# lincbrain/Fibers.jl

Hardware: AMD Instinct MI355X
Metric: Mvoxels/s fit (GQI ODF + peaks, 140^3 x 270-dir); Mpoints/s streamline in extra (higher is better)
Workload: dtype f32 (operands as 2 fp16 pieces = 23 bits on MFMA, 3 piece products, f32 accumulate); 1 GPU; gqi_rec + find_peaks + qa normalisation (gqi.jl:109-201), ONE 140x140x140 x 270-frame volume (18 x b=5 + 84 dirs x {1000,2000,3000}), sphere_642, all-ones mask; voxels=2744000, voxels_per_gpu=2744000, frames=270, odf_vertices=321, parallelism=single GPU

## Files before the change

fibers.jl_amd/csrc/odf.hip:

```cpp
#include <algorithm>
#include <cmath>
#include <type_traits>
#include <utility>

#include "common.h"

namespace {

typedef float f32x16 __attribute__((ext_vector_type(16)));

constexpr int KT = 16;
constexpr int WG_VOX = 128;

#include "odf_gemm_f32.inc"
#include "odf_fused_epilogue.inc"
#include "odf_gemm3.inc"
#include "odf_mask.inc"
#include "odf_peaks.inc"
#include "odf_post.inc"

}

struct fib_odf_plan {
    int device = 0, ncu = 256;
    int nvol = 0, nvert = 0, nrows = 0, nrow0 = 0;
    int MB = 11, NX = 0, ntile_m = 1, Kpad = 0, maxdeg = 0;
    int scale_frame = -1;
    float scale_coef = 0.0f;
    bool has_ineff = false;
    int gM = 0, gK = 0, gRow0 = 0;
    std::vector<float> G;
    bool folded = false;
    int fold_span_max = 0, scale_frame_raw = -1;
    fib::DevBuf<int32_t> foldA, foldB;
    mutable fib::DevBuf<float> folded_dwi;
    std::vector<float> A;
    fib::DevBuf<float> At, verts;
    fib::DevBuf<uint16_t> At3;
    fib::DevBuf<float> Aextra;
    fib::DevBuf<float> Gdev;
    mutable fib::DevBuf<int32_t> inf_list;
    bool split_bf16 = false;
    bool h2 = false;
    float h2_sa = 1.0f;
    bool fused_shape = false;
    bool fused = false;
    bool dsi2_shape = false, dsi2 = false;
    int MBB = 0;
    fib::DevBuf<uint16_t> At3b;
    mutable fib::DevBuf<unsigned> pair_flags;
    fib::DevBuf<uint16_t> At3f;
    fib::DevBuf<float> Aextraf;
    mutable fib::DevBuf<float> mean_hi;
    mutable fib::DevBuf<int32_t> redo_list;
    fib::DevBuf<uint32_t> effbits;
    fib::DevBuf<int32_t> nbr, nbr64;
    int deg_pad = 6, rows_pad = 0;
// ... 3 lines not shown
    mutable fib::DevBuf<unsigned long long> compact_state;
    mutable fib::DevBuf<unsigned long long> compact_sub;
    mutable fib::DevBuf<unsigned long long> compact_state2;
    mutable fib::DevBuf<unsigned> compact_mode;
    mutable fib::DevBuf<unsigned long long> compact_oct;
    mutable unsigned compact_epoch = 0;
    fib::DevBuf<unsigned> tickets;
    fib::DevBuf<unsigned> selctr;
    fib::DevBuf<unsigned long long> sellist;
    mutable fib::DevBuf<float> odfmax;
};

namespace {


int resolve_format(int format) {
    if (format != FIB_ODF_FORMAT_DEFAULT) return format;
    const char *e = fib::env("FIBERS_ODF_FORMAT");
    if (!e) {
        const char *g = fib::env("FIBERS_ODF_GEMM"), *x = fib::env("FIBERS_ODF_EXACT");
        if (g && (!strcmp(g, "f32") || !strcmp(g, "F32"))) return FIB_ODF_FORMAT_F32;
        if (x && x[0] != '\0' && x[0] != '0') return FIB_ODF_FORMAT_BF16X3;
    }
    if (e && (!strcmp(e, "f32") || !strcmp(e, "F32"))) return FIB_ODF_FORMAT_F32;
    if (e && (!strcmp(e, "bf16x3") || !strcmp(e, "BF16X3"))) return FIB_ODF_FORMAT_BF16X3;
    return FIB_ODF_FORMAT_FP16X2;
}

int finish_plan(fib_odf_plan *p, const float *verts, int nverts, const int32_t *faces, int nfaces,
                const std::vector<float> &frame_eff, int format = FIB_ODF_FORMAT_DEFAULT) {
    if (p->G.empty()) { p->G = p->A; p->gM = p->nrows; p->gK = p->nvol; p->gRow0 = p->nrow0; }
    const int M = p->gM, K = p->gK;
    if (hipDeviceGetAttribute(&p->ncu, hipDeviceAttributeMultiprocessorCount, p->device) != hipSuccess) p->ncu = 256;
    format = resolve_format(format);
    p->split_bf16 = format != FIB_ODF_FORMAT_F32;
    int best_cost = INT32_MAX;
    const int nxs[] = {0, 1};
    for (int mb = p->split_bf16 ? 10 : 11; mb >= 5; mb--)
        for (int nx : nxs) {
            if (nx > 0 && mb > 10) continue;
            const int rows = mb * 32 + nx;
            const int nt = (M + rows - 1) / rows;
            const int cost = nt * (64 * mb + 4 * nx);
            if (cost < best_cost) { best_cost = cost; p->MB = mb; p->NX = nx; p->ntile_m = nt; }
        }
    p->Kpad = (K + KT - 1) / KT * KT;
    const int MW = gemm_row_stride(p->MB, p->NX), ROWS = p->MB * 32 + p->NX;
    std::vector<float> At((size_t)p->ntile_m * p->Kpad * MW, 0.0f);
    for (int k = 0; k < K; k++)
        for (int r = 0; r < M; r++) {
            const int tm = r / ROWS, rr = r % ROWS;
            At[((size_t)tm * p->Kpad + k) * MW + rr] = p->G[r + (size_t)M * k];
        }
    bool any_ineff = false;
    for (int k = 0; k < K; k++) if (frame_eff[k] == 0.0f) any_ineff = true;
    if (p->split_bf16 && (any_ineff || p->Kpad / KT < 2 || p->MB > 10 || (size_t)p->ntile_m * p->NX * p->Kpad > 2048)) p->split_bf16 = false;
    if (p->split_bf16) {
        p->h2 = format == FIB_ODF_FORMAT_FP16X2;
        float gmax = 0.0f;
        for (float v : p->G) if (std::isfinite(v)) gmax = std::max(gmax, std::fabs(v));
        if (p->h2 && !(gmax > 0.0f)) p->h2 = false;
        for (float v : p->G) if (!std::isfinite(v)) p->h2 = false;
        if (p->h2) { int eg; std::frexp(gmax, &eg); p->h2_sa = std::ldexp(1.0f, 9 - eg); }
        const int NP = p->h2 ? 2 : 3;
        const int npiece = NP * p->MB, nst = p->Kpad / KT;
        auto f16_rn = [](float f) -> uint16_t { const _Float16 h = (_Float16)f; uint16_t u; memcpy(&u, &h, 2); return u; };
// ... 232 lines not shown
                if (fa[c] == p->scale_frame) p->scale_frame = -1000 - c;
            }
            if (p->scale_frame <= -1000) { p->scale_frame = -(p->scale_frame + 1000); p->scale_frame_raw = fa[p->scale_frame]; }
            for (int t0 = 0; t0 < nrep; t0 += KT)
                for (const std::vector<int32_t> *side : {&fa, &fb}) {
                    int lo = 1 << 30, hi = -1;
                    for (int j = t0; j < std::min(nrep, t0 + KT); j++) if ((*side)[j] >= 0) { lo = std::min(lo, (*side)[j]); hi = std::max(hi, (*side)[j]); }
                    if (hi >= 0) p->fold_span_max = std::max(p->fold_span_max, hi - lo + 1);
                }
            FIB_RC(fib::upload(p->foldA, fa));
            FIB_RC(fib::upload(p->foldB, fb));
            eff.assign((size_t)nrep, 1.0f);
        }
    }
    FIB_RC(finish_plan(p.get(), verts, nverts, faces, nfaces, eff, format));
    *plan = p.release();
    return FIB_OK;
} FIB_API_CATCH

extern "C" void fib_odf_plan_destroy(fib_odf_plan *plan) try { fib::plan_destroy(plan); } FIB_API_CATCH_VOID

extern "C" int fib_odf_plan_matrix(const fib_odf_plan *plan, float *A, int *nrows, int *nvol, int *nvert) try {
    FIB_CHECK(plan != nullptr, FIB_ERR_INVALID, "plan is NULL");
    if (nrows) *nrows = plan->nrows;
    if (nvol) *nvol = plan->nvol;
    if (nvert) *nvert = plan->nvert;
    if (A) memcpy(A, plan->A.data(), plan->A.size() * sizeof(float));
    return FIB_OK;
} FIB_API_CATCH

namespace {

constexpr int FOLD_MB_MAX = 10;
constexpr int POST_GRID = 384;

struct OdfRoute {
    bool compact = false;
    bool split = false;
    bool fused = false;
    bool dsi2 = false;
    bool fold_fused = false;
    bool fold_pre = false;
    bool fold4 = false;
    bool inf_fix = false;
    bool peaks = false;
    bool vec_ok = false;
    bool scan() const { return fused || dsi2; }
};

OdfRoute odf_route(const fib_odf_plan *plan, int64_t nvox, bool out16, bool in16, int flags) {
    OdfRoute r;
    const bool sep = (flags & FIB_ODF_SEPARATE_PEAKS) != 0;
    r.compact = true;
    r.vec_ok = out16;
    r.split = plan->split_bf16 && nvox <= ((int64_t)1 << 26);
    r.inf_fix = r.split && plan->Gdev.p != nullptr;
    r.fused = plan->fused && r.split && out16 && !sep;
    const bool fold_ok = plan->folded && r.split && plan->Kpad <= FKMAX && plan->scale_frame_raw >= 0 &&
                         (int64_t)plan->fold_span_max * nvox * 4 < (int64_t)0xE0000000ll;
    r.dsi2 = plan->dsi2 && fold_ok && out16 && !sep;
    r.fold_fused = (fold_ok && plan->MB <= FOLD_MB_MAX) || r.dsi2;
    r.fold_pre = plan->folded && !r.fold_fused;
    r.fold4 = r.fold_pre && in16;
    r.peaks = !r.scan();
    return r;
}

// ... 170 lines not shown
    return FIB_OK;
}

int launch_mask_compact(const fib_odf_plan *plan, const uint8_t *mask, int64_t nvox, unsigned *maxenc, const ZeroArgs *z, hipStream_t st) {
    int iters = (int)std::max<int64_t>(1, fib::cdiv(fib::cdiv(nvox, CB), 256));
    if (iters > CB_ITERS_MAX) iters = CB_ITERS_MAX;
    const int nchunks = (int)fib::cdiv(nvox, (int64_t)CB * iters);
    FIB_CHECK(nchunks <= 1024, FIB_ERR_UNSUPPORTED, "volume too large for the mask compaction");
    FIB_RC(fresh_zeroed(plan->compact_state, 1024, st));
    FIB_RC(fresh_zeroed(plan->compact_state2, 1024, st));
    if (!plan->compact_mode.p) {
        FIB_RC(plan->compact_mode.alloc(2));
        FIB_HIP(hipMemsetD32Async(reinterpret_cast<hipDeviceptr_t>(plan->compact_mode.p), 1, 2, st));
    }
    if (z) FIB_RC(fresh_zeroed(plan->compact_sub, (size_t)fib::cdiv(nvox, CB), st));
    if (++plan->compact_epoch == 0u) plan->compact_epoch = 1u;
    CompactArgs c{};
    c.mask = mask; c.nvox = nvox; c.vidx = plan->live_vox.p; c.tiles = plan->live_tiles.p; c.state = plan->compact_state.p;
    c.ticket = plan->tickets.p; c.totals = plan->live_counts.p; c.maxenc = maxenc; c.epoch = plan->compact_epoch; c.nchunks = nchunks; c.iters = iters;
    c.zero = z != nullptr;
    if (z) c.z = *z;
    c.clear = plan->pair_flags.p; c.nclear = plan->pair_flags.p ? 8 * 32 : 0;
    c.sub_state = plan->compact_sub.p;
    c.state2 = plan->compact_state2.p; c.mode = plan->compact_mode.p;
    const size_t noct = (size_t)fib::cdiv(nvox, 1024);
    if (z && noct * sizeof(unsigned) <= 48 * 1024) {
        FIB_RC(fresh_zeroed(plan->compact_oct, noct, st));
        c.oct_bits = plan->compact_oct.p; c.oct_words = (int)noct;
    }
    { const char *e = fib::ab_env("FIBERS_COMPACT_UNKNOWN"); c.dbg_unknown = e ? atoi(e) : 0; }
    { const char *e = fib::ab_env("FIBERS_ODF_LIST"); c.force = !e ? -1 : (e[0] == 'q' ? 0 : (e[0] == 'o' ? 1 : -1)); }
    fib::ProfScope prof("mask_compact", st);
    const int grid = nchunks + (z ? 256 : 0);
    hipLaunchKernelGGL(mask_compact_kernel, dim3(grid), dim3(1024), c.oct_words * sizeof(unsigned), st, c);
    FIB_HIP(hipGetLastError());
    return FIB_OK;
}

void launch_fold(const fib_odf_plan *plan, const OdfRoute &r, const float *dwi, const uint8_t *mask, int64_t nvox, hipStream_t st) {
    fib::ProfScope prof("dsi_fold", st);
    const unsigned grid = (unsigned)fib::cdiv(r.fold4 ? nvox / 4 : nvox, 256);
    hipLaunchKernelGGL(r.fold4 ? dsi_fold4_kernel : dsi_fold_kernel, dim3(grid), dim3(256), 0, st, dwi, mask, plan->foldA.p, plan->foldB.p,
                       plan->gK, nvox, plan->folded_dwi.p);
}

GemmArgs odf_gemm_args(const fib_odf_plan *plan, const OdfRoute &r, const float *dwi, const uint8_t *mask, float *pdf, float *odf,
                       float *const peak[3], float *const qa[3], int64_t nvox) {
    GemmArgs ga = gemm_args(plan, r, r.fold_pre ? plan->folded_dwi.p : dwi, mask, pdf, odf, nvox);
#ifdef FIB_CLOCK_STAMP
    { const char *pi = fib::ab_env("FIBERS_PHASE_ITEM"); ga.phase_item = pi ? atoi(pi) : 2; }
    { const char *pw = fib::ab_env("FIBERS_PHASE_WG"); ga.phase_wg = pw ? atoi(pw) : 8; }
#endif
    if (r.inf_fix) { ga.fix_count = plan->live_counts.p + 2; ga.fix_list = plan->inf_list.p; ga.fix_cap = (int)std::min<int64_t>(nvox, INT32_MAX); }
    if (r.scan()) add_scan_args(ga, plan, peak, qa);
    if (r.dsi2) add_dsi2_args(ga, plan);
    return ga;
}

int launch_post(const fib_odf_plan *plan, const OdfRoute &r, const GemmArgs &ga, const float *dwi, float *odf, float *const peak[3],
                float *const qa[3], int64_t nvox, float *odfmax, int flags, hipStream_t st) {
    fib::ProfScope prof("odf_post", st);
    PostArgs pa{};
    pa.redo = RedoArgs{odf, nvox, ga.redo_count, ga.redo_list, ga.redo_cap, plan->verts.p, {peak[0], peak[1], peak[2]}, {qa[0], qa[1], qa[2]}, plan->maxenc.p};
    pa.G = (r.scan() && r.inf_fix) ? plan->Gdev.p : nullptr; pa.S = dwi; pa.out = odf; pa.M = plan->gM; pa.K = plan->gK;
    pa.refine = RefineArgs{odf, nvox, nvox, plan->nvert, plan->live_vox.p, plan->live_counts.p, plan->mean_hi.p, plan->maxenc.p};
    pa.arrive = plan->tickets.p + 1; pa.odfmax = odfmax; pa.raw = (flags & FIB_ODF_RAW_ODFMAX) ? 1 : 0;
    pa.selctr = plan->selctr.p; pa.sellist = plan->sellist.p; pa.selcap = POST_SELCAP; pa.epoch = plan->compact_epoch;
    if (flags & FIB_ODF_NORMALIZE) {
        for (int k = 0; k < 3; k++) pa.nq[k] = qa[k];
        pa.nq_n = nvox; pa.done = reinterpret_cast<unsigned long long *>(plan->tickets.p + 2);
    }
    { const char *e = fib::ab_env("FIBERS_POST_SKIP"); pa.dbg = e ? atoi(e) : 0; }
    hipLaunchKernelGGL(odf_post_kernel, dim3(POST_GRID), dim3(256), 0, st, pa);
    FIB_HIP(hipGetLastError());
    return FIB_OK;
}
}

extern "C" int fibd_odf_rec(const fib_odf_plan *plan, const float *dwi, const uint8_t *mask, int64_t nvox,
                            float *pdf, float *odf, float *const peak[3], float *const qa[3],
                            float *odfmax_dev, int flags, void *stream) try {
    FIB_CHECK(plan && dwi && mask && odf && peak && qa, FIB_ERR_INVALID, "NULL argument");
    FIB_CHECK(nvox > 0, FIB_ERR_INVALID, "nvox must be positive");
    FIB_CHECK(nvox <= ((int64_t)1 << 27), FIB_ERR_UNSUPPORTED, "volumes of more than 2^27 voxels are not supported (32-bit lane offsets)");
    FIB_CHECK(plan->nrow0 == 0 || pdf != nullptr, FIB_ERR_INVALID, "DSI plans need a pdf output volume");
    for (int k = 0; k < 3; k++) FIB_CHECK(peak[k] && qa[k], FIB_ERR_INVALID, "NULL peak/qa output volume");
    FIB_CHECK(fib::cdiv(nvox, WG_VOX) * plan->ntile_m < ((int64_t)1 << 31), FIB_ERR_UNSUPPORTED, "volume too large for one launch");
    fib::DeviceGuard guard;
    FIB_HIP(hipSetDevice(plan->device));
    hipStream_t st = (hipStream_t)stream;
    const bool out16 = nvox % 4 == 0 && ((uintptr_t)odf & 15) == 0 && (pdf == nullptr || ((uintptr_t)pdf & 15) == 0);
    const bool in16 = nvox % 4 == 0 && ((uintptr_t)dwi & 15) == 0 && ((uintptr_t)mask & 3) == 0;
    const OdfRoute route = odf_route(plan, nvox, out16, in16, flags);
    FIB_RC(odf_scratch(plan, route, nvox));
    ZeroArgs z{};
    z.out0 = pdf; z.out1 = odf; z.n0 = plan->nrow0; z.n1 = plan->nrows - plan->nrow0; z.nvox = nvox; z.stride = nvox;
    for (int k = 0; k < 3; k++) { z.peak[k] = peak[k]; z.qa[k] = qa[k]; }
    FIB_RC(launch_mask_compact(plan, mask, nvox, plan->maxenc.p, !(flags & FIB_ODF_PREZEROED) ? &z : nullptr, st));
    if (route.fold_pre) launch_fold(plan, route, dwi, mask, nvox, st);
    const GemmArgs ga = odf_gemm_args(plan, route, dwi, mask, pdf, odf, peak, qa, nvox);
    FIB_RC(launch_contraction(plan, route, ga, "odf_gemm", st));
    if (route.peaks) {
        if (route.inf_fix) {
            InfFixArgs fx{plan->Gdev.p, dwi, odf, ga.fix_count, ga.fix_list, ga.fix_cap, plan->gM, plan->gK, nvox};
            hipLaunchKernelGGL(odf_inf_fix_kernel, dim3(64), dim3(256), 0, st, fx);
        }
        FIB_RC(launch_peaks(plan, odf, nvox, nvox, peak, qa, nullptr, nullptr, true, st, false, plan->live_tiles.p, plan->live_counts.p + 1));
// ... 48 lines not shown

extern "C" int fibd_qa_normalize_dev(float *const qa[3], int64_t nvox, const float *odfmax_dev, void *stream) try {
    FIB_CHECK(qa && qa[0] && qa[1] && qa[2] && odfmax_dev && nvox > 0, FIB_ERR_INVALID, "NULL argument");
    return qa_normalize(qa, nvox, const_cast<float *>(odfmax_dev), 0.0f, 0, stream);
} FIB_API_CATCH

extern "C" int fibd_qa_normalize_pair(float *const qa[3], int64_t nvox, float *odfmax_pair_dev, void *stream) try {
    FIB_CHECK(qa && qa[0] && qa[1] && qa[2] && odfmax_pair_dev && nvox > 0, FIB_ERR_INVALID, "NULL argument");
    return qa_normalize(qa, nvox, odfmax_pair_dev, 0.0f, 1, stream);
} FIB_API_CATCH

extern "C" int fibd_find_peaks(const fib_odf_plan *plan, const float *odf, int64_t nvox,
                               int32_t *isort_top, int32_t *nvalid, void *stream) try {
    FIB_CHECK(plan && odf && isort_top && nvalid && nvox > 0, FIB_ERR_INVALID, "NULL argument");
    fib::DeviceGuard guard;
    FIB_HIP(hipSetDevice(plan->device));
    return launch_peaks(plan, odf, nvox, nvox, nullptr, nullptr, isort_top, nvalid, false, (hipStream_t)stream);
} FIB_API_CATCH

#ifdef FIB_CLOCK_STAMP
extern "C" int fib_debug_clock_stamps(unsigned long long *out, int cap) try {
    FIB_CHECK(out && cap > 0 && cap <= 2048, FIB_ERR_INVALID, "invalid stamp buffer");
    FIB_HIP(hipDeviceSynchronize());
    FIB_HIP(hipMemcpyFromSymbol(out, HIP_SYMBOL(fib_clock_stamps), (size_t)cap * 4 * sizeof(unsigned long long), 0, hipMemcpyDeviceToHost));
    return FIB_OK;
} FIB_API_CATCH
extern "C" int fib_debug_phase_stamps(unsigned long long *out) try {
    FIB_CHECK(out, FIB_ERR_INVALID, "invalid stamp buffer");
    FIB_HIP(hipDeviceSynchronize());
    FIB_HIP(hipMemcpyFromSymbol(out, HIP_SYMBOL(fib_phase_stamps), sizeof(unsigned long long) * 512, 0, hipMemcpyDeviceToHost));
    return FIB_OK;
} FIB_API_CATCH

extern "C" int fib_debug_clock_clear(void) try {
    static unsigned long long zeros[2048][4];
    FIB_HIP(hipMemcpyToSymbol(HIP_SYMBOL(fib_clock_stamps), zeros, sizeof(zeros), 0, hipMemcpyHostToDevice));
    return FIB_OK;
} FIB_API_CATCH
#endif

extern "C" int fibd_find_peaks_work(const fib_odf_plan *plan, const float *odf, int64_t nvox,
                                    float *odf_peak, int32_t *isort, int32_t *nvalid, void *stream) try {
    FIB_CHECK(plan && odf && odf_peak && isort && nvalid && nvox > 0, FIB_ERR_INVALID, "NULL argument");
    FIB_CHECK(plan->nbr64.p != nullptr && plan->maxdeg > 0, FIB_ERR_INVALID, "the plan has no tessellation");
    fib::DeviceGuard guard;
    FIB_HIP(hipSetDevice(plan->device));
    const size_t smem = (size_t)plan->nvert * sizeof(unsigned long long) + (size_t)(plan->nvert + 1) * sizeof(float);
    FIB_CHECK(smem <= 64 * 1024, FIB_ERR_UNSUPPORTED, "ODF with %d vertices does not fit the peak finder's LDS", plan->nvert);
    const unsigned grid = (unsigned)std::min<int64_t>(nvox, 8192);
    hipLaunchKernelGGL(odf_peaks_work_kernel, dim3(grid), dim3(256), smem, (hipStream_t)stream, odf, nvox, nvox, plan->nvert, plan->deg_pad,
                       plan->nbr64.p, odf_peak, isort, nvalid);
    FIB_HIP(hipGetLastError());
    return FIB_OK;
} FIB_API_CATCH
```

fibers.jl_amd/csrc/odf_mask.inc:

```

constexpr int CB = 4096;
constexpr int CB_ITERS_MAX = 32;
__device__ __forceinline__ unsigned long long quad_expand(unsigned long long b) {
    unsigned long long q = (b | (b >> 1) | (b >> 2) | (b >> 3)) & 0x1111111111111111ull;
    return q | (q << 1) | (q << 2) | (q << 3);
}
__device__ __forceinline__ unsigned long long octet_expand(unsigned long long b) {
    return ((b & 0xffffffffull) ? 0xffffffffull : 0ull) | ((b >> 32) ? 0xffffffff00000000ull : 0ull);
}
struct ZeroArgs { float *out0, *out1, *peak[3], *qa[3]; int n0, n1; int64_t nvox, stride; };
struct CompactArgs {
    const uint8_t *mask; int64_t nvox;
    int32_t *vidx, *tiles;
    unsigned long long *state;
    unsigned *ticket;
    int32_t *totals;
    unsigned *maxenc;
    unsigned epoch;
    int nchunks, iters, zero;
    unsigned *clear; int nclear;
    unsigned long long *sub_state;
    unsigned long long *state2;
    unsigned *mode;
    int force;
    unsigned long long *oct_bits;
    int oct_words;
    int dbg_unknown;
    ZeroArgs z;
};
typedef __attribute__((address_space(1))) unsigned long long fib_gu64;
__global__ __launch_bounds__(1024) void mask_compact_kernel(const CompactArgs c) {
    __shared__ int cv[CB_ITERS_MAX][64], ct[CB_ITERS_MAX][64];
    __shared__ int s_chunk, s_base[2], s_agg[2], s_ndead[CB_ITERS_MAX], s_oct, s_alt[2], s_altsum[2];
    __shared__ unsigned s_gbits[CB_ITERS_MAX * 4];
    extern __shared__ unsigned s_octbits[];
    const int tid = threadIdx.x, lane = tid & 63, wave = tid >> 6;
    const bool compacts = (int)blockIdx.x < c.nchunks;
    if (compacts) {
        if (tid == 0) {
            s_chunk = (int)atomicAdd(c.ticket, 1u); s_base[0] = 0; s_base[1] = 0; s_alt[0] = 0; s_alt[1] = 0; s_altsum[0] = 0; s_altsum[1] = 0;
            s_oct = c.force >= 0 ? c.force : (c.mode ? (int)(c.mode[c.epoch & 1u] != 0u) : 0);
        }
        if (tid < CB_ITERS_MAX) s_ndead[tid] = 0;
        if (tid < CB_ITERS_MAX * 4) s_gbits[tid] = 0u;
        __syncthreads();
        const int t = s_chunk;
        const bool oct = s_oct != 0;
        const int64_t base = (int64_t)t * c.iters * CB;
        int nq = 0, no = 0;
        for (int it = 0; it < c.iters; it++) {
            int nd = 0;
#pragma unroll
            for (int i = 0; i < 4; i++) {
                const int64_t vx = base + (int64_t)it * CB + i * 1024 + tid;
                const unsigned long long inr = __ballot(vx < c.nvox);
                const unsigned long long b = __ballot(vx < c.nvox && c.mask[vx] != 0);
                const unsigned long long eq = quad_expand(b) & inr, eo = octet_expand(b) & inr;
                const unsigned long long e = oct ? eo : eq;
                nd += __popcll(inr & ~b);
                nq += __popcll(eq); no += __popcll(eo);
                if (lane == 0) { cv[it][i * 16 + wave] = __popcll(e); ct[it][i * 16 + wave] = b != 0ull; }
                if (lane == 0 && b) atomicOr(&s_gbits[it * 4 + i], (((b & 0xffffffffull) ? 1u : 0u) | ((b >> 32) ? 2u : 0u)) << (2 * wave));
            }
            if (c.zero && lane == 0 && nd) atomicAdd(&s_ndead[it], nd);
        }
        if (lane == 0 && c.state2) { atomicAdd(&s_alt[0], nq); atomicAdd(&s_alt[1], no); }
        __syncthreads();
        if (c.zero && oct && c.oct_bits && tid < c.iters * 4) {
            const int64_t gi = (base + (int64_t)(tid >> 2) * CB + (int64_t)(tid & 3) * 1024) >> 10;
            if (gi < c.oct_words)
                __hip_atomic_store((fib_gu64 *)(c.oct_bits + gi), ((unsigned long long)c.epoch << 32) | (unsigned long long)s_gbits[tid], __ATOMIC_RELAXED, __HIP_MEMORY_SCOPE_AGENT);
        }
        if (tid == 0 && c.state2)
            __hip_atomic_store((fib_gu64 *)(c.state2 + t), ((unsigned long long)(c.epoch & 0xfffffffu) << 36) | ((unsigned long long)s_alt[0] << 18) | (unsigned long long)s_alt[1],
                               __ATOMIC_RELAXED, __HIP_MEMORY_SCOPE_AGENT);
        if (c.zero && tid < c.iters && (int64_t)(t * c.iters + tid) * CB < c.nvox)
            __hip_atomic_store((fib_gu64 *)(c.sub_state + (size_t)t * c.iters + tid), ((unsigned long long)c.epoch << 32) | (unsigned)s_ndead[tid],
                               __ATOMIC_RELAXED, __HIP_MEMORY_SCOPE_AGENT);
        if (wave == 0) {
            int runv = 0, runt = 0;
            for (int it = 0; it < c.iters; it++) {
                const int v = cv[it][lane], tl = ct[it][lane];
                int sv = v, stl = tl;
#pragma unroll
                for (int off = 1; off < 64; off <<= 1) {
                    const int ov = __shfl_up(sv, off), ot = __shfl_up(stl, off);
                    if (lane >= off) { sv += ov; stl += ot; }
                }
                cv[it][lane] = runv + sv - v; ct[it][lane] = runt + stl - tl;
                runv += __shfl(sv, 63); runt += __shfl(stl, 63);
            }
            if (lane == 0) {
                s_agg[0] = runv; s_agg[1] = runt;
                __hip_atomic_store((fib_gu64 *)(c.state + t), ((unsigned long long)c.epoch << 32) | ((unsigned long long)runt << 18) | (unsigned long long)runv,
                                   __ATOMIC_RELAXED, __HIP_MEMORY_SCOPE_AGENT);
            }
        }
        {
            int pv = 0, pt = 0;
            if (tid < t) {
                unsigned long long g;
                for (;;) {
                    g = __hip_atomic_load((fib_gu64 *)(c.state + tid), __ATOMIC_RELAXED, __HIP_MEMORY_SCOPE_AGENT);
                    if ((unsigned)(g >> 32) == c.epoch) break;
                    __builtin_amdgcn_s_sleep(1);
                }
                pv = (int)(g & 0x3ffffull); pt = (int)((g >> 18) & 0x3fffull);
            }
#pragma unroll
            for (int off = 32; off >= 1; off >>= 1) { pv += __shfl_xor(pv, off); pt += __shfl_xor(pt, off); }
            if (lane == 0 && (pv | pt)) { atomicAdd(&s_base[0], pv); atomicAdd(&s_base[1], pt); }
        }
        if (t == c.nchunks - 1 && c.state2 && c.mode) {
            int aq = 0, ao = 0;
            if (tid <= t) {
                unsigned long long g;
                for (;;) {
                    g = __hip_atomic_load((fib_gu64 *)(c.state2 + tid), __ATOMIC_RELAXED, __HIP_MEMORY_SCOPE_AGENT);
                    if ((unsigned)(g >> 36) == (c.epoch & 0xfffffffu)) break;
                    __builtin_amdgcn_s_sleep(1);
                }
                aq = (int)((g >> 18) & 0x3ffffull); ao = (int)(g & 0x3ffffull);
            }
#pragma unroll
            for (int off = 32; off >= 1; off >>= 1) { aq += __shfl_xor(aq, off); ao += __shfl_xor(ao, off); }
            if (lane == 0 && (aq | ao)) { atomicAdd(&s_altsum[0], aq); atomicAdd(&s_altsum[1], ao); }
        }
        __syncthreads();
        if (t == c.nchunks - 1 && wave == 0) {
            if (lane == 0 && c.state2 && c.mode) c.mode[(c.epoch + 1u) & 1u] = (2ll * s_altsum[1] <= 3ll * s_altsum[0]) ? 1u : 0u;
            if (lane == 0) {
                c.totals[0] = s_base[0] + s_agg[0]; c.totals[1] = s_base[1] + s_agg[1]; c.totals[2] = 0; c.totals[3] = 0;
                if (c.maxenc) { c.maxenc[0] = 0u; c.maxenc[1] = 0u; c.maxenc[2] = 0u; c.maxenc[3] = 0u; }
                c.ticket[0] = 0u; c.ticket[1] = 0u;
            }
            for (int i = lane; i < c.nclear; i += 64) c.clear[i] = 0u;
        }
        for (int it = 0; it < c.iters; it++)
#pragma unroll
            for (int i = 0; i < 4; i++) {
                const int64_t vx = base + (int64_t)it * CB + i * 1024 + tid;
                const unsigned long long b = __ballot(vx < c.nvox && c.mask[vx] != 0);
                const unsigned long long e = (oct ? octet_expand(b) : quad_expand(b)) & __ballot(vx < c.nvox);
                const int pv = s_base[0] + cv[it][i * 16 + wave], pt = s_base[1] + ct[it][i * 16 + wave];
                if ((e >> lane) & 1ull) c.vidx[pv + __popcll(e & ((1ull << lane) - 1ull))] = (int32_t)vx;
                if (lane == 0 && b) c.tiles[pt] = (int32_t)(vx >> 6);
            }
        if (!c.zero) return;
    }
    const ZeroArgs &z = c.z;
    constexpr int ZS = 8, ZR = 16;
    __shared__ int s_nd[ZS], s_known, s_tot[2];
    const int nr = z.n0 + z.n1 + 12, ngrp = (nr + ZR - 1) / ZR;
    const int64_t nsub = (c.nvox + CB - 1) / CB, nspan = (nsub + ZS - 1) / ZS;
    const int hb = (int)blockIdx.x, nh = (int)gridDim.x;
    if (tid < 2) s_tot[tid] = 0;
    __syncthreads();
    {
        long long nd = 0;
        int unknown = 0;
        for (int64_t sidx = tid; sidx < nsub; sidx += 1024) {
            int got = -1;
            for (int spin = 0; spin < 600; spin++) {
                const unsigned long long w = __hip_atomic_load((fib_gu64 *)(c.sub_state + sidx), __ATOMIC_RELAXED, __HIP_MEMORY_SCOPE_AGENT);
                if ((unsigned)(w >> 32) == c.epoch) { got = (int)(unsigned)w; break; }
                __builtin_amdgcn_s_sleep(4);
            }
            if (got < 0) unknown = 1; else nd += got;
        }
        int q = (int)nd;
        for (int off = 32; off >= 1; off >>= 1) { q += __shfl_xor(q, off); unknown |= __shfl_xor(unknown, off); }
        if (lane == 0) { atomicAdd(&s_tot[0], q); if (unknown) atomicOr(&s_tot[1], 1); }
    }
    __syncthreads();
    const bool all_known = s_tot[1] == 0 && !(c.dbg_unknown > 0 && (int)blockIdx.x % c.dbg_unknown == 1);
    const int64_t total_dead = s_tot[0];
    if (all_known && total_dead == 0) return;
    const bool whole_ok = z.stride == c.nvox && (c.nvox & 3) == 0;
    const bool whole = all_known && total_dead * 4 > c.nvox && whole_ok;
    const bool both = !all_known && whole_ok;
    if (whole || both) {
        const bool octs = c.oct_bits != nullptr && c.oct_words > 0 && (c.force >= 0 ? c.force != 0 : (c.mode != nullptr && c.mode[c.epoch & 1u] != 0u));
        if (octs) {
            for (int gi = tid; gi < c.oct_words; gi += 1024) {
                unsigned bits = 0u;
                for (int spin = 0; spin < 600; spin++) {
                    const unsigned long long w = __hip_atomic_load((fib_gu64 *)(c.oct_bits + gi), __ATOMIC_RELAXED, __HIP_MEMORY_SCOPE_AGENT);
                    if ((unsigned)(w >> 32) == c.epoch) { bits = (unsigned)w; break; }
                    __builtin_amdgcn_s_sleep(4);
                }
                s_octbits[gi] = bits;
            }
            __syncthreads();
        }
        const int64_t nqrow = c.nvox >> 2;
        auto clear_rows = [&](float *p, int nrows) {
            if (!p || nrows <= 0) return;
            typedef float v4f __attribute__((ext_vector_type(4)));
            const v4f zero4 = {0.f, 0.f, 0.f, 0.f};
            v4f *d = reinterpret_cast<v4f *>(p);
            const int64_t nq = (int64_t)nrows * nqrow, step = (int64_t)nh * 4096;
            int64_t q = (int64_t)hb * 4096 + tid;
            int64_t qi = q % nqrow;
            const int64_t srow = step % nqrow;
            for (; q < nq; q += step) {
                int64_t qk = qi;
#pragma unroll
// ... 157 lines not shown
```

fibers.jl_amd/csrc/odf_post.inc:

```

__device__ __forceinline__ unsigned long long wave_max_u64(unsigned long long k) {
    for (int off = 32; off >= 1; off >>= 1) {
        const unsigned lo = (unsigned)__shfl_xor((int)(unsigned)k, off), hi = (unsigned)__shfl_xor((int)(unsigned)(k >> 32), off);
        const unsigned long long o = ((unsigned long long)hi << 32) | lo;
        k = o > k ? o : k;
    }
    return k;
}
constexpr int POST_SELCAP = 2048;
struct RedoArgs { const float *odf; int64_t stride; const int32_t *count, *list; int cap; const float *verts; float *peak[3], *qa[3]; unsigned *maxenc; };
struct RefineArgs { const float *odf; int64_t stride, nvox; int nvert; const int32_t *vidx, *nlive; const float *mean_hi; unsigned *maxenc; };
struct PostArgs {
    RedoArgs redo;
    const float *G, *S; float *out; int M, K;
    RefineArgs refine;
    unsigned *arrive;
    float *odfmax;
    int raw;
    float *nq[3]; int64_t nq_n;
    unsigned long long *done;
    unsigned epoch;
    unsigned *selctr;
    unsigned long long *sellist;
    int selcap;
// ... 22 lines not shown
    for (int k = 0; k < 3; k++) {
        const unsigned long long m = wave_max_u64(t.k[0]);
        best.k[k] = m;
        if (m != 0ull && t.k[0] == m) { t.k[0] = t.k[1]; t.k[1] = t.k[2]; t.k[2] = 0ull; }
    }
    for (int off = 32; off >= 1; off >>= 1) {
        npos += __shfl_xor(npos, off);
        const float om = __shfl_xor(vmin, off);
        vmin = om < vmin ? om : vmin;
    }
    if (__any(hasnan)) vmin = __builtin_nanf("");
    if (lane == 0) {
        float sum = 0.0f;
        for (int v = 0; v < NV; v++) sum += o[v];
        const float mean = sum / (float)NV;
        if (mean != mean) atomicOr(&a.maxenc[1], 1u); else atomicMax(&a.maxenc[0], enc_ordered(mean));
        const int n3 = npos < 3 ? npos : 3;
#pragma unroll
        for (int k = 0; k < 3; k++) {
            float px = 0.0f, py = 0.0f, pz = 0.0f, q = 0.0f;
            if (k < n3) {
                const int iv = top3_index(best, k);
                px = a.verts[3 * iv]; py = a.verts[3 * iv + 1]; pz = a.verts[3 * iv + 2];
                q = o[iv] - vmin;
            }
            a.peak[k][vox] = px; a.peak[k][a.stride + vox] = py; a.peak[k][2 * a.stride + vox] = pz;
            a.qa[k][vox] = q;
        }
    }
}
__global__ __launch_bounds__(256) void odf_post_kernel(const PostArgs p) {
    __shared__ float col[4][512];
    const int lane = threadIdx.x & 63, wv = threadIdx.x >> 6;
    if (p.redo.count && !(p.dbg & 1)) {
        constexpr int NV = FIB_S642_NVERT;
        const RedoArgs &a = p.redo;
        float *o = col[wv];
        const int n = a.count[0] < a.cap ? a.count[0] : a.cap;
        for (int i = blockIdx.x * 4 + wv; i < n; i += gridDim.x * 4) {
            const unsigned ent = (unsigned)a.list[i];
            const int64_t vox = (int64_t)(ent & 0x7fffffffu);
            __builtin_amdgcn_wave_barrier();
            if ((ent >> 31) && p.G) {
                for (int row = lane; row < p.M; row += 64) {
                    float acc = 0.0f;
                    for (int k = 0; k < p.K; k++) acc = __builtin_fmaf(p.G[row + (size_t)p.M * k], clamp_sample(p.S[(int64_t)k * a.stride + vox]), acc);
                    p.out[(int64_t)row * a.stride + vox] = acc;
                    if (row < NV) o[row] = acc;
                }
            } else {
                for (int v = lane; v < NV; v += 64) o[v] = a.odf[(int64_t)v * a.stride + vox];
            }
            if (lane == 0) o[NV] = __builtin_nanf("");
            __builtin_amdgcn_wave_barrier();
            redo_voxel(a, o, vox, lane);
        }
        __builtin_amdgcn_wave_barrier();
        if (n > 0 && p.nq[0]) __builtin_amdgcn_fence(__ATOMIC_RELEASE, "agent");
    }
    if (!(p.dbg & 2)) {
        const RefineArgs &a = p.refine;
        const int nlive = a.nlive[0];
        if (blockIdx.x == 0 && threadIdx.x == 0 && nlive < a.nvox) atomicMax(&a.maxenc[0], enc_ordered(0.0f));
        const unsigned lo_e = a.maxenc[2];
        const float m_lo = lo_e ? dec_ordered(lo_e) : -INFINITY;
        const bool ident = (int64_t)nlive == a.nvox;
        constexpr int PU = 4;
        const int64_t nquad = ((int64_t)nlive + 3) / 4, nth = (int64_t)gridDim.x * 256, nround = (nquad + 64 * PU - 1) / (64 * PU) * (64 * PU);
        unsigned ebest = 0u;
        auto column_mean = [&](int64_t v) {
            if (a.nvert <= 512) {
                for (int r = lane; r < a.nvert; r += 64) col[wv][r] = a.odf[(int64_t)r * a.stride + v];
                __builtin_amdgcn_wave_barrier();
                if (lane == 0) {
                    float sum = 0.0f;
                    for (int r = 0; r < a.nvert; r++) sum += col[wv][r];
                    const unsigned e = enc_ordered(sum / (float)a.nvert);
                    ebest = e > ebest ? e : ebest;
                }
                __builtin_amdgcn_wave_barrier();
            } else if (lane == 0) {
                float sum = 0.0f;
                for (int r = 0; r < a.nvert; r++) sum += a.odf[(int64_t)r * a.stride + v];
                const unsigned e = enc_ordered(sum / (float)a.nvert);
                ebest = e > ebest ? e : ebest;
            }
        };
        for (int64_t q0 = ((int64_t)blockIdx.x * 256 + (threadIdx.x & ~63)) * PU + lane; q0 < nround; q0 += nth * PU) {
            int64_t vq[PU];
            float mhu[PU][4];
#pragma unroll
            for (int u = 0; u < PU; u++) {
// ... 6 lines not shown
                mhu[u][0] = mhu[u][1] = mhu[u][2] = mhu[u][3] = -INFINITY;
                if (q < nquad) {
                    if (4 * q + 4 <= nlive && (vox0 & 3) == 0) {
                        const float4 m4 = *reinterpret_cast<const float4 *>(a.mean_hi + vox0);
                        mhu[u][0] = m4.x; mhu[u][1] = m4.y; mhu[u][2] = m4.z; mhu[u][3] = m4.w;
                    } else {
                        for (int j = 0; j < 4; j++) if (4 * q + j < nlive) mhu[u][j] = a.mean_hi[ident ? 4 * q + j : (int64_t)a.vidx[4 * q + j]];
                    }
                }
            }
#pragma unroll
            for (int u = 0; u < PU; u++) {
                const int64_t q = q0 + 64 * u, vox0 = vq[u];
#pragma unroll
                for (int j = 0; j < 4; j++) {
                    const bool sel = 4 * q + j < nlive && mhu[u][j] >= m_lo && !(p.dbg & 8);
                    const int64_t vox = (4 * q + 4 <= nlive && (vox0 & 3) == 0) ? vox0 + j : (sel ? (ident ? 4 * q + j : (int64_t)a.vidx[4 * q + j]) : 0);
                    bool here = false;
                    if (sel) {
                        const unsigned slot = __hip_atomic_fetch_add(p.selctr + 1, 1u, __ATOMIC_RELAXED, __HIP_MEMORY_SCOPE_AGENT);
                        if (slot < (unsigned)p.selcap)
                            __hip_atomic_store((fib_gu64 *)(p.sellist + slot), ((unsigned long long)p.epoch << 32) | (unsigned long long)(unsigned)vox, __ATOMIC_RELAXED, __HIP_MEMORY_SCOPE_AGENT);
                        else here = true;
                    }
                    unsigned long long todo = __ballot(here);
                    while (todo) {
                        const int src = __ffsll((long long)todo) - 1;
                        todo &= todo - 1ull;
                        column_mean(__shfl(vox, src));
                    }
                }
            }
        }
        for (;;) {
            int vsel = -1;
            if (lane == 0) {
                for (;;) {
                    unsigned h = __hip_atomic_load(p.selctr, __ATOMIC_RELAXED, __HIP_MEMORY_SCOPE_AGENT);
                    unsigned t = __hip_atomic_load(p.selctr + 1, __ATOMIC_RELAXED, __HIP_MEMORY_SCOPE_AGENT);
                    t = t < (unsigned)p.selcap ? t : (unsigned)p.selcap;
                    if (h >= t) break;
                    if (__hip_atomic_compare_exchange_strong(p.selctr, &h, h + 1u, __ATOMIC_RELAXED, __ATOMIC_RELAXED, __HIP_MEMORY_SCOPE_AGENT)) {
                        unsigned long long g;
                        for (;;) {
                            g = __hip_atomic_load((fib_gu64 *)(p.sellist + h), __ATOMIC_RELAXED, __HIP_MEMORY_SCOPE_AGENT);
                            if ((unsigned)(g >> 32) == p.epoch) break;
                            __builtin_amdgcn_s_sleep(1);
                        }
                        vsel = (int)(unsigned)g;
                        break;
                    }
                }
            }
            vsel = __shfl(vsel, 0);
            if (vsel < 0) break;
            column_mean((int64_t)vsel);
        }
        if (lane == 0 && ebest) atomicMax(&a.maxenc[0], ebest);
    }
    asm volatile("s_waitcnt vmcnt(0)" ::: "memory");
    __syncthreads();
    if (threadIdx.x == 0) {
        const unsigned old = __hip_atomic_fetch_add(p.arrive, 1u, __ATOMIC_RELAXED, __HIP_MEMORY_SCOPE_AGENT);
        if (old == gridDim.x - 1) {
            const unsigned e0 = __hip_atomic_load(&p.refine.maxenc[0], __ATOMIC_RELAXED, __HIP_MEMORY_SCOPE_AGENT);
            const unsigned e1 = __hip_atomic_load(&p.refine.maxenc[1], __ATOMIC_RELAXED, __HIP_MEMORY_SCOPE_AGENT);
            const bool nan = e1 != 0;
            const float m = e0 ? dec_ordered(e0) : -INFINITY;
            const float d = nan ? NAN : m;
            p.odfmax[0] = (p.nq[0] || !p.raw) ? d : m;
            p.odfmax[1] = nan ? 1.0f : 0.0f;
            __hip_atomic_store(p.arrive, 0u, __ATOMIC_RELAXED, __HIP_MEMORY_SCOPE_AGENT);
            __hip_atomic_store(p.selctr, 0u, __ATOMIC_RELAXED, __HIP_MEMORY_SCOPE_AGENT);
            __hip_atomic_store(p.selctr + 1, 0u, __ATOMIC_RELAXED, __HIP_MEMORY_SCOPE_AGENT);
            if (p.nq[0])
                __hip_atomic_store((fib_gu64 *)p.done, ((unsigned long long)p.epoch << 32) | (unsigned long long)__float_as_uint(d), __ATOMIC_RELAXED, __HIP_MEMORY_SCOPE_AGENT);
        }
    }
    if (!p.nq[0]) return;
    __shared__ float s_d;
    if (threadIdx.x == 0) {
        unsigned long long g;
        for (;;) {
            g = __hip_atomic_load((fib_gu64 *)p.done, __ATOMIC_RELAXED, __HIP_MEMORY_SCOPE_AGENT);
            if ((unsigned)(g >> 32) == p.epoch) break;
            __builtin_amdgcn_s_sleep(2);
        }
        s_d = __uint_as_float((unsigned)g);
    }
    __syncthreads();
    const float d = s_d;
    if (p.dbg & 4) return;
    if (p.redo.count && p.redo.count[0] > 0) __builtin_amdgcn_fence(__ATOMIC_ACQUIRE, "agent");
    const int64_t t0 = (int64_t)blockIdx.x * 256 + threadIdx.x, nt = (int64_t)gridDim.x * 256;
    if ((p.nq_n & 3) == 0 && ((reinterpret_cast<uintptr_t>(p.nq[0]) | reinterpret_cast<uintptr_t>(p.nq[1]) | reinterpret_cast<uintptr_t>(p.nq[2])) & 15) == 0) {
        const int64_t n4 = p.nq_n >> 2;
        for (int k = 0; k < 3; k++) {
            float4 *q4 = reinterpret_cast<float4 *>(p.nq[k]);
            for (int64_t i0 = t0; i0 < n4; i0 += nt * 8) {
                float4 v[8];
#pragma unroll
                for (int j = 0; j < 8; j++) if (i0 + j * nt < n4) v[j] = q4[i0 + j * nt];
#pragma unroll
                for (int j = 0; j < 8; j++)
                    if (i0 + j * nt < n4) {
                        v[j].x = v[j].x / d; v[j].y = v[j].y / d; v[j].z = v[j].z / d; v[j].w = v[j].w / d;
                        q4[i0 + j * nt] = v[j];
                    }
            }
        }
    } else {
        for (int64_t i = t0; i < p.nq_n; i += nt) {
            p.nq[0][i] = p.nq[0][i] / d; p.nq[1][i] = p.nq[1][i] / d; p.nq[2][i] = p.nq[2][i] / d;
        }
    }
}

__global__ __launch_bounds__(256) void qa_normalize_kernel(float *q0, float *q1, float *q2, int64_t nvox,
                                                          float *odfmax_dev, float odfmax_val, int pair) {
    float d = odfmax_dev ? odfmax_dev[0] : odfmax_val;
    if (pair) {
        d = odfmax_dev[1] > 0.0f ? NAN : d;
        if (blockIdx.x == 0 && threadIdx.x == 0) odfmax_dev[0] = d;
    }
    for (int64_t i = (int64_t)blockIdx.x * blockDim.x + threadIdx.x; i < nvox; i += (int64_t)gridDim.x * blockDim.x) {
        q0[i] = q0[i] / d;
        q1[i] = q1[i] / d;
        q2[i] = q2[i] / d;
    }
}

__global__ __launch_bounds__(256) void odf_peaks_work_kernel(const float *__restrict__ odf, int64_t stride, int64_t nvox, int nvert, int deg,
                                                             const int32_t *__restrict__ nbr64, float *__restrict__ odf_peak,
                                                             int32_t *__restrict__ isort, int32_t *__restrict__ nvalid) {
    extern __shared__ __attribute__((aligned(16))) unsigned long long pk_keys[];
    float *o = reinterpret_cast<float *>(pk_keys + nvert);
    __shared__ int cnt;
    for (int64_t vox = blockIdx.x; vox < nvox; vox += gridDim.x) {
        __syncthreads();
        for (int v = threadIdx.x; v < nvert; v += blockDim.x) o[v] = odf[(int64_t)v * stride + vox];
        if (threadIdx.x == 0) { o[nvert] = __builtin_nanf(""); cnt = 0; }
        __syncthreads();
        int mine = 0;
        for (int v = threadIdx.x; v < nvert; v += blockDim.x) {
            const float x = o[v];
            bool killed = false;
            for (int d = 0; d < deg; d++) killed |= o[nbr64[(size_t)v * deg + d]] >= x;
            const float pk = killed ? 0.0f : x;
// ... 16 lines not shown
```

Baseline: 1512 Mvoxels/s.

## Vectorize mask compaction by quads, template iteration count, guard fused post normalization

```diff
diff --git a/fibers.jl_amd/csrc/odf.hip b/fibers.jl_amd/csrc/odf.hip
--- a/fibers.jl_amd/csrc/odf.hip
+++ b/fibers.jl_amd/csrc/odf.hip
@@ -11,6 +11,7 @@
 
 constexpr int KT = 16;
 constexpr int WG_VOX = 128;
+constexpr int POST_GRID = 384;
 
 #include "odf_gemm_f32.inc"
 #include "odf_fused_epilogue.inc"
@@ -23,6 +24,7 @@
 
 struct fib_odf_plan {
     int device = 0, ncu = 256;
+    bool post_resident = false;
     int nvol = 0, nvert = 0, nrows = 0, nrow0 = 0;
     int MB = 11, NX = 0, ntile_m = 1, Kpad = 0, maxdeg = 0;
     int scale_frame = -1;
@@ -92,6 +94,11 @@
     if (p->G.empty()) { p->G = p->A; p->gM = p->nrows; p->gK = p->nvol; p->gRow0 = p->nrow0; }
     const int M = p->gM, K = p->gK;
     if (hipDeviceGetAttribute(&p->ncu, hipDeviceAttributeMultiprocessorCount, p->device) != hipSuccess) p->ncu = 256;
+    {
+        int per_cu = 0;
+        p->post_resident = hipOccupancyMaxActiveBlocksPerMultiprocessor(&per_cu, odf_post_kernel, 256, 0) == hipSuccess &&
+                           (int64_t)per_cu * p->ncu >= POST_GRID;
+    }
     format = resolve_format(format);
     p->split_bf16 = format != FIB_ODF_FORMAT_F32;
     int best_cost = INT32_MAX;
@@ -390,7 +397,6 @@
 namespace {
 
 constexpr int FOLD_MB_MAX = 10;
-constexpr int POST_GRID = 384;
 
 struct OdfRoute {
     bool compact = false;
@@ -627,7 +633,7 @@
     { const char *e = fib::ab_env("FIBERS_ODF_LIST"); c.force = !e ? -1 : (e[0] == 'q' ? 0 : (e[0] == 'o' ? 1 : -1)); }
     fib::ProfScope prof("mask_compact", st);
     const int grid = nchunks + (z ? 256 : 0);
-    hipLaunchKernelGGL(mask_compact_kernel, dim3(grid), dim3(1024), c.oct_words * sizeof(unsigned), st, c);
+    hipLaunchKernelGGL(iters <= 4 ? mask_compact_kernel<4> : mask_compact_kernel<CB_ITERS_MAX>, dim3(grid), dim3(1024), c.oct_words * sizeof(unsigned), st, c);
     FIB_HIP(hipGetLastError());
     return FIB_OK;
 }
@@ -654,20 +660,27 @@
 
 int launch_post(const fib_odf_plan *plan, const OdfRoute &r, const GemmArgs &ga, const float *dwi, float *odf, float *const peak[3],
                 float *const qa[3], int64_t nvox, float *odfmax, int flags, hipStream_t st) {
+    const char *enorm = fib::ab_env("FIBERS_POST_NORM");
+    const bool norm = (flags & FIB_ODF_NORMALIZE) != 0, norm_fused = norm && plan->post_resident && !(enorm && enorm[0] == 's');
     fib::ProfScope prof("odf_post", st);
     PostArgs pa{};
     pa.redo = RedoArgs{odf, nvox, ga.redo_count, ga.redo_list, ga.redo_cap, plan->verts.p, {peak[0], peak[1], peak[2]}, {qa[0], qa[1], qa[2]}, plan->maxenc.p};
     pa.G = (r.scan() && r.inf_fix) ? plan->Gdev.p : nullptr; pa.S = dwi; pa.out = odf; pa.M = plan->gM; pa.K = plan->gK;
     pa.refine = RefineArgs{odf, nvox, nvox, plan->nvert, plan->live_vox.p, plan->live_counts.p, plan->mean_hi.p, plan->maxenc.p};
-    pa.arrive = plan->tickets.p + 1; pa.odfmax = odfmax; pa.raw = (flags & FIB_ODF_RAW_ODFMAX) ? 1 : 0;
+    pa.arrive = plan->tickets.p + 1; pa.odfmax = odfmax;
+    pa.raw = ((flags & FIB_ODF_RAW_ODFMAX) && !norm) ? 1 : 0;
     pa.selctr = plan->selctr.p; pa.sellist = plan->sellist.p; pa.selcap = POST_SELCAP; pa.epoch = plan->compact_epoch;
-    if (flags & FIB_ODF_NORMALIZE) {
+    if (norm_fused) {
         for (int k = 0; k < 3; k++) pa.nq[k] = qa[k];
         pa.nq_n = nvox; pa.done = reinterpret_cast<unsigned long long *>(plan->tickets.p + 2);
     }
     { const char *e = fib::ab_env("FIBERS_POST_SKIP"); pa.dbg = e ? atoi(e) : 0; }
     hipLaunchKernelGGL(odf_post_kernel, dim3(POST_GRID), dim3(256), 0, st, pa);
     FIB_HIP(hipGetLastError());
+    if (norm && !norm_fused) {
+        hipLaunchKernelGGL(qa_normalize_kernel, dim3(2048), dim3(256), 0, st, qa[0], qa[1], qa[2], nvox, odfmax, 0.0f, 0);
+        FIB_HIP(hipGetLastError());
+    }
     return FIB_OK;
 }
 }
@@ -782,6 +795,13 @@
     return FIB_OK;
 } FIB_API_CATCH
 
+extern "C" int fib_debug_side_stamps(unsigned long long *out) try {
+    FIB_CHECK(out, FIB_ERR_INVALID, "invalid stamp buffer");
+    FIB_HIP(hipDeviceSynchronize());
+    FIB_HIP(hipMemcpyFromSymbol(out, HIP_SYMBOL(fib_side_stamps), sizeof(unsigned long long) * 2 * 512 * 8, 0, hipMemcpyDeviceToHost));
+    return FIB_OK;
+} FIB_API_CATCH
+
 extern "C" int fib_debug_clock_clear(void) try {
     static unsigned long long zeros[2048][4];
     FIB_HIP(hipMemcpyToSymbol(HIP_SYMBOL(fib_clock_stamps), zeros, sizeof(zeros), 0, hipMemcpyHostToDevice));
diff --git a/fibers.jl_amd/csrc/odf_mask.inc b/fibers.jl_amd/csrc/odf_mask.inc
--- a/fibers.jl_amd/csrc/odf_mask.inc
+++ b/fibers.jl_amd/csrc/odf_mask.inc
@@ -1,12 +1,27 @@
 
 constexpr int CB = 4096;
+#ifdef FIB_CLOCK_STAMP
+__device__ unsigned long long fib_side_stamps[2][512][8];
+#define FIB_SIDE_MARK(k_, id_)                                                                                                      \
+    do {                                                                                                                            \
+        unsigned long long t_;                                                                                                      \
+        asm volatile("s_memrealtime %0\n\ts_waitcnt lgkmcnt(0)" : "=s"(t_) :: "memory");                                            \
+        if (threadIdx.x == 0 && blockIdx.x < 512) fib_side_stamps[k_][blockIdx.x][id_] = t_;                                        \
+    } while (0)
+#else
+#define FIB_SIDE_MARK(k_, id_) do { } while (0)
+#endif
 constexpr int CB_ITERS_MAX = 32;
-__device__ __forceinline__ unsigned long long quad_expand(unsigned long long b) {
-    unsigned long long q = (b | (b >> 1) | (b >> 2) | (b >> 3)) & 0x1111111111111111ull;
-    return q | (q << 1) | (q << 2) | (q << 3);
-}
-__device__ __forceinline__ unsigned long long octet_expand(unsigned long long b) {
-    return ((b & 0xffffffffull) ? 0xffffffffull : 0ull) | ((b >> 32) ? 0xffffffff00000000ull : 0ull);
+__device__ __forceinline__ unsigned mask_quad(const uint8_t *mask, int64_t v0, int64_t nvox, bool al4) {
+    if (al4 && v0 + 4 <= nvox) return *reinterpret_cast<const unsigned *>(mask + v0);
+    unsigned w = 0u;
+    for (int j = 0; j < 4; j++) if (v0 + j < nvox) w |= (unsigned)(mask[v0 + j] != 0) << (8 * j);
+    return w;
+}
+__device__ __forceinline__ unsigned long long octet_expand_quads(unsigned long long q) {
+    unsigned long long t = q | (q >> 1);
+    t |= t >> 2; t |= t >> 4;
+    return (t & 0x0101010101010101ull) * 0xffull;
 }
 struct ZeroArgs { float *out0, *out1, *peak[3], *qa[3]; int n0, n1; int64_t nvox, stride; };
 struct CompactArgs {
@@ -29,43 +44,64 @@
     ZeroArgs z;
 };
 typedef __attribute__((address_space(1))) unsigned long long fib_gu64;
+template <int ITM>
 __global__ __launch_bounds__(1024) void mask_compact_kernel(const CompactArgs c) {
-    __shared__ int cv[CB_ITERS_MAX][64], ct[CB_ITERS_MAX][64];
-    __shared__ int s_chunk, s_base[2], s_agg[2], s_ndead[CB_ITERS_MAX], s_oct, s_alt[2], s_altsum[2];
-    __shared__ unsigned s_gbits[CB_ITERS_MAX * 4];
+    __shared__ int cv[ITM][64], ct[ITM][64];
+    __shared__ int s_chunk, s_base[2], s_agg[2], s_ndead[ITM], s_oct, s_alt[2], s_altsum[2];
+    __shared__ unsigned s_gbits[ITM * 4];
     extern __shared__ unsigned s_octbits[];
     const int tid = threadIdx.x, lane = tid & 63, wave = tid >> 6;
     const bool compacts = (int)blockIdx.x < c.nchunks;
+    FIB_SIDE_MARK(0, 0);
     if (compacts) {
         if (tid == 0) {
             s_chunk = (int)atomicAdd(c.ticket, 1u); s_base[0] = 0; s_base[1] = 0; s_alt[0] = 0; s_alt[1] = 0; s_altsum[0] = 0; s_altsum[1] = 0;
             s_oct = c.force >= 0 ? c.force : (c.mode ? (int)(c.mode[c.epoch & 1u] != 0u) : 0);
         }
-        if (tid < CB_ITERS_MAX) s_ndead[tid] = 0;
-        if (tid < CB_ITERS_MAX * 4) s_gbits[tid] = 0u;
+        if (tid < ITM) s_ndead[tid] = 0;
+        if (tid < ITM * 4) s_gbits[tid] = 0u;
         __syncthreads();
         const int t = s_chunk;
+        FIB_SIDE_MARK(0, 1);
         const bool oct = s_oct != 0;
         const int64_t base = (int64_t)t * c.iters * CB;
+        const bool al4 = (reinterpret_cast<uintptr_t>(c.mask) & 3) == 0;
+        const int part = (int)(c.nvox & 3);
+        unsigned mw[ITM];
+#pragma unroll
+        for (int it = 0; it < ITM; it++) mw[it] = it < c.iters ? mask_quad(c.mask, base + (int64_t)it * CB + tid * 4, c.nvox, al4) : 0u;
         int nq = 0, no = 0;
-        for (int it = 0; it < c.iters; it++) {
-            int nd = 0;
-#pragma unroll
-            for (int i = 0; i < 4; i++) {
-                const int64_t vx = base + (int64_t)it * CB + i * 1024 + tid;
-                const unsigned long long inr = __ballot(vx < c.nvox);
-                const unsigned long long b = __ballot(vx < c.nvox && c.mask[vx] != 0);
-                const unsigned long long eq = quad_expand(b) & inr, eo = octet_expand(b) & inr;
-                const unsigned long long e = oct ? eo : eq;
-                nd += __popcll(inr & ~b);
-                nq += __popcll(eq); no += __popcll(eo);
-                if (lane == 0) { cv[it][i * 16 + wave] = __popcll(e); ct[it][i * 16 + wave] = b != 0ull; }
-                if (lane == 0 && b) atomicOr(&s_gbits[it * 4 + i], (((b & 0xffffffffull) ? 1u : 0u) | ((b >> 32) ? 2u : 0u)) << (2 * wave));
-            }
-            if (c.zero && lane == 0 && nd) atomicAdd(&s_ndead[it], nd);
+#pragma unroll
+        for (int it = 0; it < ITM; it++) {
+            if (it >= c.iters) continue;
+            const int64_t v0 = base + (int64_t)it * CB + tid * 4;
+            const int nin = v0 + 4 <= c.nvox ? 4 : (v0 < c.nvox ? (int)(c.nvox - v0) : 0);
+            const unsigned w = mw[it];
+            const unsigned long long Q = __ballot(w != 0u), R = __ballot(nin > 0), P = __ballot(nin > 0 && nin < 4);
+            auto listed = [&](unsigned long long E) { return 4 * __popcll(E) - ((E & P) ? 4 - part : 0); };
+            const unsigned long long eq = Q, eo = octet_expand_quads(Q) & R;
+            const unsigned long long e = oct ? eo : eq;
+            nq += listed(eq); no += listed(eo);
+            if (lane < 4) {
+                const unsigned long long tm = 0xffffull << (16 * lane);
+                cv[it][wave * 4 + lane] = listed(e & tm); ct[it][wave * 4 + lane] = (Q & tm) != 0ull;
+            }
+            if (lane == 0 && Q) {
+                unsigned o8 = 0u;
+#pragma unroll
+                for (int o = 0; o < 8; o++) o8 |= (((Q >> (8 * o)) & 0xffull) ? 1u : 0u) << o;
+                atomicOr(&s_gbits[it * 4 + (wave >> 2)], o8 << (8 * (wave & 3)));
+            }
+            if (c.zero) {
+                const int nins = __popcll(__ballot((w & 0xffu) != 0u)) + __popcll(__ballot((w & 0xff00u) != 0u)) +
+                                 __popcll(__ballot((w & 0xff0000u) != 0u)) + __popcll(__ballot((w & 0xff000000u) != 0u));
+                const int nd = listed(R) - nins;
+                if (lane == 0 && nd) atomicAdd(&s_ndead[it], nd);
+            }
         }
         if (lane == 0 && c.state2) { atomicAdd(&s_alt[0], nq); atomicAdd(&s_alt[1], no); }
         __syncthreads();
+        FIB_SIDE_MARK(0, 2);
         if (c.zero && oct && c.oct_bits && tid < c.iters * 4) {
             const int64_t gi = (base + (int64_t)(tid >> 2) * CB + (int64_t)(tid & 3) * 1024) >> 10;
             if (gi < c.oct_words)
@@ -127,6 +163,7 @@
             if (lane == 0 && (aq | ao)) { atomicAdd(&s_altsum[0], aq); atomicAdd(&s_altsum[1], ao); }
         }
         __syncthreads();
+        FIB_SIDE_MARK(0, 3);
         if (t == c.nchunks - 1 && wave == 0) {
             if (lane == 0 && c.state2 && c.mode) c.mode[(c.epoch + 1u) & 1u] = (2ll * s_altsum[1] <= 3ll * s_altsum[0]) ? 1u : 0u;
             if (lane == 0) {
@@ -136,16 +173,25 @@
             }
             for (int i = lane; i < c.nclear; i += 64) c.clear[i] = 0u;
         }
-        for (int it = 0; it < c.iters; it++)
-#pragma unroll
-            for (int i = 0; i < 4; i++) {
-                const int64_t vx = base + (int64_t)it * CB + i * 1024 + tid;
-                const unsigned long long b = __ballot(vx < c.nvox && c.mask[vx] != 0);
-                const unsigned long long e = (oct ? octet_expand(b) : quad_expand(b)) & __ballot(vx < c.nvox);
-                const int pv = s_base[0] + cv[it][i * 16 + wave], pt = s_base[1] + ct[it][i * 16 + wave];
-                if ((e >> lane) & 1ull) c.vidx[pv + __popcll(e & ((1ull << lane) - 1ull))] = (int32_t)vx;
-                if (lane == 0 && b) c.tiles[pt] = (int32_t)(vx >> 6);
-            }
+        const bool val16 = (reinterpret_cast<uintptr_t>(c.vidx) & 15) == 0;
+#pragma unroll
+        for (int it = 0; it < ITM; it++) {
+            if (it >= c.iters) continue;
+            const int64_t v0 = base + (int64_t)it * CB + tid * 4;
+            const int nin = v0 + 4 <= c.nvox ? 4 : (v0 < c.nvox ? (int)(c.nvox - v0) : 0);
+            const unsigned long long Q = __ballot(mw[it] != 0u), R = __ballot(nin > 0);
+            const unsigned long long e = oct ? octet_expand_quads(Q) & R : Q;
+            const int pv = s_base[0] + cv[it][wave * 4] + 4 * __popcll(e & ((1ull << lane) - 1ull));
+            if ((e >> lane) & 1ull) {
+                if (nin == 4 && val16 && (pv & 3) == 0) {
+                    *reinterpret_cast<int4 *>(c.vidx + pv) = make_int4((int)v0, (int)v0 + 1, (int)v0 + 2, (int)v0 + 3);
+                } else {
+                    for (int j = 0; j < nin; j++) c.vidx[pv + j] = (int32_t)(v0 + j);
+                }
+            }
+            if ((lane & 15) == 0 && (Q & (0xffffull << lane))) c.tiles[s_base[1] + ct[it][wave * 4 + (lane >> 4)]] = (int32_t)(v0 >> 6);
+        }
+        FIB_SIDE_MARK(0, 4);
         if (!c.zero) return;
     }
     const ZeroArgs &z = c.z;
@@ -173,6 +219,7 @@
         if (lane == 0) { atomicAdd(&s_tot[0], q); if (unknown) atomicOr(&s_tot[1], 1); }
     }
     __syncthreads();
+    FIB_SIDE_MARK(0, 5);
     const bool all_known = s_tot[1] == 0 && !(c.dbg_unknown > 0 && (int)blockIdx.x % c.dbg_unknown == 1);
     const int64_t total_dead = s_tot[0];
     if (all_known && total_dead == 0) return;
diff --git a/fibers.jl_amd/csrc/odf_post.inc b/fibers.jl_amd/csrc/odf_post.inc
--- a/fibers.jl_amd/csrc/odf_post.inc
+++ b/fibers.jl_amd/csrc/odf_post.inc
@@ -78,6 +78,7 @@
 __global__ __launch_bounds__(256) void odf_post_kernel(const PostArgs p) {
     __shared__ float col[4][512];
     const int lane = threadIdx.x & 63, wv = threadIdx.x >> 6;
+    FIB_SIDE_MARK(1, 0);
     if (p.redo.count && !(p.dbg & 1)) {
         constexpr int NV = FIB_S642_NVERT;
         const RedoArgs &a = p.redo;
@@ -104,6 +105,7 @@
         __builtin_amdgcn_wave_barrier();
         if (n > 0 && p.nq[0]) __builtin_amdgcn_fence(__ATOMIC_RELEASE, "agent");
     }
+    FIB_SIDE_MARK(1, 1);
     if (!(p.dbg & 2)) {
         const RefineArgs &a = p.refine;
         const int nlive = a.nlive[0];
@@ -176,6 +178,7 @@
                 }
             }
         }
+        FIB_SIDE_MARK(1, 2);
         for (;;) {
             int vsel = -1;
             if (lane == 0) {
@@ -204,6 +207,7 @@
     }
     asm volatile("s_waitcnt vmcnt(0)" ::: "memory");
     __syncthreads();
+    FIB_SIDE_MARK(1, 3);
     if (threadIdx.x == 0) {
         const unsigned old = __hip_atomic_fetch_add(p.arrive, 1u, __ATOMIC_RELAXED, __HIP_MEMORY_SCOPE_AGENT);
         if (old == gridDim.x - 1) {
@@ -221,6 +225,7 @@
                 __hip_atomic_store((fib_gu64 *)p.done, ((unsigned long long)p.epoch << 32) | (unsigned long long)__float_as_uint(d), __ATOMIC_RELAXED, __HIP_MEMORY_SCOPE_AGENT);
         }
     }
+    FIB_SIDE_MARK(1, 4);
     if (!p.nq[0]) return;
     __shared__ float s_d;
     if (threadIdx.x == 0) {
@@ -234,6 +239,7 @@
     }
     __syncthreads();
     const float d = s_d;
+    FIB_SIDE_MARK(1, 5);
     if (p.dbg & 4) return;
     if (p.redo.count && p.redo.count[0] > 0) __builtin_amdgcn_fence(__ATOMIC_ACQUIRE, "agent");
     const int64_t t0 = (int64_t)blockIdx.x * 256 + threadIdx.x, nt = (int64_t)gridDim.x * 256;
@@ -258,6 +264,10 @@
             p.nq[0][i] = p.nq[0][i] / d; p.nq[1][i] = p.nq[1][i] / d; p.nq[2][i] = p.nq[2][i] / d;
         }
     }
+#ifdef FIB_CLOCK_STAMP
+    asm volatile("s_waitcnt vmcnt(0)" ::: "memory");
+#endif
+    FIB_SIDE_MARK(1, 6);
 }
 
 __global__ __launch_bounds__(256) void qa_normalize_kernel(float *q0, float *q1, float *q2, int64_t nvox,
```

Result: slower. 1490 Mvoxels/s (-1.4%).
